# DeepRec-AI/HybridBackend

Measured on AMD Instinct MI355X. Metric: M-lookups/sec, 26-col Criteo-shape dim16, 1/2/4/8 GPUs; % HBM roofline, higher is better.
Workload: dtype f32

## Files before the change

hybridbackend_amd/csrc/common.h:

```cpp
#ifndef HBK_CSRC_COMMON_H_
#define HBK_CSRC_COMMON_H_

#include <hip/hip_runtime.h>
#include <stdarg.h>
#include <stdint.h>
#include <stdio.h>

#include "hbk.h"

namespace hbk {

int fail(int code, const char* fmt, ...);

#define HBK_HIP_OK(expr)                                                         \
  do {                                                                           \
    hipError_t e__ = (expr);                                                     \
    if (e__ != hipSuccess) {                                                     \
      return ::hbk::fail(HBK_INTERNAL, "%s failed: %s (%s:%d)", #expr,           \
                         hipGetErrorString(e__), __FILE__, __LINE__);            \
    }                                                                            \
  } while (0)

#define HBK_REQUIRE(cond, ...)                                                   \
  do {                                                                           \
// ... 45 lines not shown
  unsigned __int128 num = (unsigned __int128)1 << (64 + k);
  uint64_t m = (uint64_t)(num / d);
  uint64_t rem = (uint64_t)(num % d);
  uint64_t m2 = m * 2;
  uint64_t twice_rem = rem * 2;
  if (twice_rem >= d || twice_rem < rem) m2 += 1;
  f.magic = m2 + 1;
  f.shift = k;
  f.kind = 2;
  return f;
}

__host__ __device__ inline uint64_t mulhi64(uint64_t a, uint64_t b) {
#if defined(__HIP_DEVICE_COMPILE__)
  return __umul64hi(a, b);
#else
  return (uint64_t)(((unsigned __int128)a * b) >> 64);
#endif
}

__host__ __device__ inline uint64_t fastdiv(uint64_t n, const FastDiv& f) {
  if (f.kind == 0) return n;
  if (f.kind == 1) return n >> f.shift;
  uint64_t t = mulhi64(f.magic, n);
  return (((n - t) >> 1) + t) >> f.shift;
}

__host__ __device__ inline uint64_t fastmod(uint64_t n, const FastDiv& f) {
  if (f.kind == 0) return 0;
  if (f.kind == 1) return n & (f.d - 1);
  return n - fastdiv(n, f) * f.d;
}

__host__ __device__ inline int xcd_contiguous(int b, int n, int on) {
  if (!on) return b;
  const int q = n >> 3, r = n & 7, x = b & 7, i = b >> 3;
  return (x < r ? x * (q + 1) : r * (q + 1) + (x - r) * q) + i;
}


__host__ __device__ inline uint64_t floormod_i64(int64_t v, const FastDiv& f) {
  uint64_t u = v < 0 ? (uint64_t)(~v) : (uint64_t)v;
  uint64_t r = fastmod(u, f);
  return v < 0 ? f.d - 1 - r : r;
}

struct Options {
  int bwd_buckets_log2 = -1;
  int bwd_bucket_pairs = 0;
  int bwd_split_pairs = 0;
  int bwd_onepass = 1;
  int fwd_xcd = 1;
  int bwd_xcd = 1;
  int bwd_wide = 1;
  int bwd_group_cols = 0;
  int bwd_dense = 1;
  int bwd_scatter_staged = 1;
  int bwd_rowsort_pos = 64;
  int bwd_pairs_packed = 1;
  int bwd_seg_inline = 1;
  int bwd_scale_fused = 1;
  int bwd_deterministic = 0;
  int bwd_simple = 1;
  int bwd_streams = 4;
  int bwd_lds_pad = 0;
  int bwd_trace = 0;
  int bwd_large_first = 0;
  int bwd_rowsort_ratio = 8;
  int bwd_weights_lds = 1;
  int fwd_d16 = 1;
  int fwd_interleave = 2;
  int fwd_hot_rows = 0;
  int unique_buckets_log2 = -1;
  int partition_sub_tiles = 1;
  int partition_fixed_max = 8;
  int partition_onepass = 1;
  int unique_onepass = 1;
  int sharded_groups = 0;
  int sharded_id64 = 0;
  int sharded_copy_self = 0;
  int sharded_trace = 0;
  int sharded_pack_early = 1;
  int sharded_wire_fused = 1;
  int sharded_inline = 1;
  int sharded_p2p = 1;
  int sharded_p2p_test_refuse = -1;
  int sync_wait_ms = 2000;
  int sync_onepass_off = 0;
  int sync_test_withhold = -1;
};
Options& options();

struct SyncTake {
  int32_t* words;
  int32_t* zero;
  int64_t zero_words;
  int32_t* status;
  int32_t* summary;
  int32_t* poison;
  unsigned long long wait_ticks;
  int32_t withhold;
};
struct SyncWait {
  int32_t* status;
  int32_t* summary;
  int32_t* poison;
  unsigned long long ticks;
  int32_t withhold;
  int32_t pad_;
};
inline SyncWait sync_wait_of(const SyncTake& t) {
  SyncWait w;
  w.status = t.status;
  w.summary = t.summary;
  w.poison = t.poison;
  w.ticks = t.wait_ticks;
  w.withhold = t.withhold;
  w.pad_ = 0;
  return w;
}
#define HBK_SYNC_SAME_STREAM (reinterpret_cast<hipStream_t>(~(uintptr_t)0))
bool sync_take(hipStream_t stream, size_t words, SyncTake* out, const void* kernel = nullptr,
               int block = 0, int max_column_wgs = 0, hipStream_t owner = HBK_SYNC_SAME_STREAM);
class SyncChain {
 public:
  explicit SyncChain(hipStream_t stream);
  ~SyncChain();
  SyncChain(const SyncChain&) = delete;
  SyncChain& operator=(const SyncChain&) = delete;

 private:
  hipStream_t stream_;
  void* state_;
};
int sync_check(const char* who, hipStream_t stream);
int sync_check_any(const char* who);

struct SlotNames {
  const char* who;
  const char* opt;
  const char* s0;
  const char* s1;
};
int adam_check(const hbk_adam_t* adam, float lr, const char* who);
int ftrl_check(const hbk_ftrl_t* ftrl, float lr, const char* who);

int bwd_check(int32_t n_cols, const hbk_lookup_grad_column_t* cols, int32_t apply, float apply_lr);

struct WeightGradColumn {
  const float* table;
  int64_t rows;
  int32_t dim;
  int32_t table_pitch;
  int32_t ids_dtype;
  const void* ids;
  int64_t n_ids;
  const int32_t* row_splits;
  int64_t n_segments;
  int64_t bucket;
  int32_t divisor;
  int32_t combiner;
  const float* grad_out;
  int32_t grad_stride;
  const float* id_weights;
  float max_norm;
  float* grad_weights;
// ... 32 lines not shown
```

hybridbackend_amd/csrc/lookup_fwd.hip:

```cpp
#include <stdlib.h>
#include <string.h>

#include <vector>

#include "lookup_common.h"

namespace hbk {
namespace {

constexpr int kBlock = 256;
constexpr int kWavesPerBlock = kBlock / kWave;
constexpr int kMaxColsPerLaunch = 128;
constexpr int kU = 2;
constexpr int kSegIters = 4;

struct ColArg {
  const float* table;
  const void* ids;
  const int32_t* splits;
  float* out;
  int64_t n_seg;
  IdMap map;
  int32_t dim;
  int32_t chunks;
  uint8_t lpr_log2;
  uint8_t ids64;
  uint8_t combiner;
  uint8_t vec4;
  int32_t n_runs;
  int32_t out_stride;
  const int64_t* run_start;
  const int64_t* run_base;
  union {
    const int32_t* out_slots;
    const float* weights;
  };
};

template <bool RUNS>
__device__ inline uint64_t row_offset(const ColArg& c, uint64_t r) {
  if (!RUNS) return r * (uint64_t)c.dim;
  int k = 0;
  while (k + 1 < c.n_runs && (uint64_t)c.run_start[k + 1] <= r) ++k;
  return (uint64_t)c.run_base[k] + (r - (uint64_t)c.run_start[k]) * (uint64_t)c.dim;
}

template <typename V, int HALF>
__device__ inline void store_out_chunk(float* out, int64_t off, V v) {
  if (HALF != 1) {
    __builtin_nontemporal_store(v, reinterpret_cast<V*>(out + off));
    return;
  }
  _Float16* o = reinterpret_cast<_Float16*>(out) + off;
  if (sizeof(V) == 16) {
    const f32x4 f = *reinterpret_cast<const f32x4*>(&v);
    const f16x4 h = {(_Float16)f[0], (_Float16)f[1], (_Float16)f[2], (_Float16)f[3]};
    __builtin_nontemporal_store(h, reinterpret_cast<f16x4*>(o));
  } else {
    *o = (_Float16)*reinterpret_cast<const float*>(&v);
  }
}

struct LookupArgs {
  int32_t n_cols;
  int32_t hot_mode;
  int32_t xcd;
  int32_t interleave;
  int32_t tile_start[kMaxColsPerLaunch + 1];
  ColArg col[kMaxColsPerLaunch];
};
static_assert(sizeof(LookupArgs) <= 24576, "kernarg budget");

template <typename V, int U, bool RUNS, int HALF, bool SLOT = false, bool D16 = false, bool WGT = false,
          bool CLIP = false>
__device__ inline void gather_rows(const ColArg& c, int64_t wave_row0, float max_norm = 0.0f) {
  constexpr int VE = sizeof(V) / 4;
  const int lane = lane_id();
  const int lpr_log2 = D16 ? 2 : c.lpr_log2;
  const int rpi = kWave >> lpr_log2;
  const int sub = lane & ((1 << lpr_log2) - 1);
  const int grp = lane >> lpr_log2;
  const int64_t n_seg = c.n_seg;

  uint64_t rowreg[U];
  int32_t slotreg[U];
  float wreg[U];
  const int n_slots = U * rpi;
#pragma unroll
  for (int k = 0; k < U; ++k) {
    rowreg[k] = kNoRow;
    slotreg[k] = 0;
    wreg[k] = 0.f;
    const int q = k * kWave + lane;
    const int64_t s = wave_row0 + q;
    if (q < n_slots && s < n_seg) {
      rowreg[k] = id_to_row(c.map, load_id(c.ids, D16 ? 1 : c.ids64, s));
      if (SLOT) slotreg[k] = __builtin_nontemporal_load(c.out_slots + s);
      if (WGT) wreg[k] = __builtin_nontemporal_load(c.weights + s);
    }
  }

  V v[U];
  const bool live = D16 ? true : sub < c.chunks;
#pragma unroll
  for (int u = 0; u < U; ++u) {
    const int q0 = u * rpi;
    const int k = q0 >> 6;
    uint64_t src = rowreg[0];
#pragma unroll
    for (int kk = 1; kk < U; ++kk) src = (k == kk) ? rowreg[kk] : src;
    const uint64_t r = shfl_u64(src, (q0 & (kWave - 1)) + grp);
    v[u] = zero_v<V>();
    if (live && r != kNoRow) {
      v[u] = load_row_chunk<V, HALF>(c.table, row_offset<RUNS>(c, r) + (uint64_t)sub * VE);
    }
    if (CLIP) v[u] = clip_row<V>(v[u], max_norm, lpr_log2);
    if (WGT) {
      float w = wreg[0];
#pragma unroll
      for (int kk = 1; kk < U; ++kk) w = (k == kk) ? wreg[kk] : w;
      w = __shfl(w, (q0 & (kWave - 1)) + grp, kWave);
      const float div = c.combiner == HBK_COMBINER_MEAN    ? w
                        : c.combiner == HBK_COMBINER_SQRTN ? sqrtf(w * w)
                                                           : 1.f;
      if (r != kNoRow && div != 0.f) {
        v[u] = v[u] * w;
        if (c.combiner != HBK_COMBINER_SUM) v[u] = v[u] / div;
      } else {
        v[u] = zero_v<V>();
      }
    }
  }
#pragma unroll
  for (int u = 0; u < U; ++u) {
    const int64_t s = wave_row0 + u * rpi + grp;
    int64_t dst = s;
    if (SLOT) {
      const int q0 = u * rpi;
      const int k = q0 >> 6;
      int32_t src = slotreg[0];
#pragma unroll
      for (int kk = 1; kk < U; ++kk) src = (k == kk) ? slotreg[kk] : src;
      dst = (int64_t)__shfl(src, (q0 & (kWave - 1)) + grp, kWave);
    }
    if (live && s < n_seg) {
      store_out_chunk<V, HALF>(c.out, dst * (int64_t)c.out_stride + (int64_t)sub * VE, v[u]);
    }
  }
}

template <typename V, bool RUNS, int HALF, bool WGT = false, bool CLIP = false>
__device__ inline void combine_segments(const ColArg& c, int64_t wave_seg0, float max_norm = 0.0f) {
  constexpr int VE = sizeof(V) / 4;
  const int lane = lane_id();
  const int lpr_log2 = c.lpr_log2;
  const int lpr = 1 << lpr_log2;
  const int rpi = kWave >> lpr_log2;
  const int sub = lane & (lpr - 1);
  const int grp = lane >> lpr_log2;
  const int grp_lane0 = grp << lpr_log2;
  const int64_t n_seg = c.n_seg;
  const bool live = sub < c.chunks;

  for (int it = 0; it < kSegIters; ++it) {
    const int64_t s = wave_seg0 + (int64_t)it * rpi + grp;
    int32_t beg = 0, end = 0;
    if (s < n_seg) {
      beg = c.splits[s];
      end = c.splits[s + 1];
    }
    V acc = zero_v<V>();
    float wsum = 0.f;
    int32_t j0 = beg;
    uint64_t myrow = kNoRow;
    float myw = 0.f;
    if (j0 + sub < end) {
      myrow = id_to_row(c.map, load_id(c.ids, c.ids64, j0 + sub));
      if (WGT) myw = __builtin_nontemporal_load(c.weights + j0 + sub);
    }
    while (__any(j0 < end)) {
      uint64_t nextrow = kNoRow;
      float nextw = 0.f;
      const int32_t j1 = j0 + lpr;
      if (j1 + sub < end) {
        nextrow = id_to_row(c.map, load_id(c.ids, c.ids64, j1 + sub));
        if (WGT) nextw = __builtin_nontemporal_load(c.weights + j1 + sub);
      }
      const int32_t cnt = end - j0;
      for (int t0 = 0; t0 < lpr; t0 += 4) {
        V v[4];
        bool p[4];
        float w[4];
#pragma unroll
        for (int t = 0; t < 4; ++t) {
          const int tt = t0 + t;
          const uint64_t r = shfl_u64(myrow, grp_lane0 + (tt & (lpr - 1)));
          p[t] = tt < lpr && tt < cnt;
          if (WGT) {
            w[t] = __shfl(myw, grp_lane0 + (tt & (lpr - 1)), kWave);
            p[t] = p[t] && r != kNoRow;
          }
          v[t] = zero_v<V>();
          if (p[t] && live && r != kNoRow) {
            v[t] = load_row_chunk<V, HALF>(c.table, row_offset<RUNS>(c, r) + (uint64_t)sub * VE);
          }
          if (CLIP) v[t] = clip_row<V>(v[t], max_norm, lpr_log2);
        }
#pragma unroll
        for (int t = 0; t < 4; ++t) {
          if (WGT) {
            if (p[t]) {
              acc = acc + v[t] * w[t];
              wsum = wsum + (c.combiner == HBK_COMBINER_SQRTN ? w[t] * w[t] : w[t]);
            }
          } else {
            if (p[t]) acc = acc + v[t];
          }
        }
      }
      myrow = nextrow;
      if (WGT) myw = nextw;
      j0 = j1;
    }
    const int32_t n = end - beg;
    if (WGT) {
      if (c.combiner != HBK_COMBINER_SUM) {
        const float div = c.combiner == HBK_COMBINER_MEAN ? wsum : sqrtf(wsum);
        acc = div != 0.f ? acc / div : zero_v<V>();
      }
    } else if (n > 0 && c.combiner == HBK_COMBINER_MEAN) {
      acc = acc / (float)n;
    } else if (n > 0 && c.combiner == HBK_COMBINER_SQRTN) {
      acc = acc / sqrtf((float)n);
    }
    if (live && s < n_seg) {
      store_out_chunk<V, HALF>(c.out, s * (int64_t)c.out_stride + (int64_t)sub * VE, acc);
    }
  }
}

template <bool CSR, typename V, bool RUNS, int HALF = 0, bool SLOT = false, bool D16 = false>
__global__ __launch_bounds__(kBlock) void group_lookup_fwd_kernel(const LookupArgs a) {
  const int b = xcd_contiguous((int)blockIdx.x, (int)gridDim.x, a.xcd);
  int ci;
  int64_t tile;
  if (a.interleave) {
    ci = b % a.n_cols;
    tile = b / a.n_cols;
  } else {
    const int lane = (int)threadIdx.x & (kWave - 1);
    const int n = a.n_cols;
    const int t0 = lane < n ? a.tile_start[lane] : 0x7fffffff;
    const int t1 = lane + kWave < n ? a.tile_start[lane + kWave] : 0x7fffffff;
    ci = (int)__builtin_popcountll(__ballot(t0 <= b)) +
         (int)__builtin_popcountll(__ballot(t1 <= b)) - 1;
    ci = __builtin_amdgcn_readfirstlane(ci);
    tile = b - a.tile_start[ci];
  }
  const ColArg& c = a.col[ci];
  const int wave = (int)(threadIdx.x >> 6);
  const int rpi = D16 ? 16 : kWave >> c.lpr_log2;
  if (!CSR) {
    const int64_t row0 = (tile * kWavesPerBlock + wave) * (int64_t)(kU * rpi);
    if (row0 >= c.n_seg) return;
    gather_rows<V, kU, RUNS, HALF, SLOT, D16>(c, row0);
  } else {
    const int64_t seg0 = (tile * kWavesPerBlock + wave) * (int64_t)(kSegIters * rpi);
    if (seg0 >= c.n_seg) return;
    combine_segments<V, RUNS, HALF>(c, seg0);
  }
}

template <bool CSR, typename V, bool RUNS, int HALF>
__global__ __launch_bounds__(kBlock) void group_lookup_fwd_weighted_kernel(const LookupArgs a) {
  const int b = xcd_contiguous((int)blockIdx.x, (int)gridDim.x, a.xcd);
  int ci;
  int64_t tile;
  if (a.interleave) {
    ci = b % a.n_cols;
    tile = b / a.n_cols;
  } else {
    const int lane = (int)threadIdx.x & (kWave - 1);
    const int n = a.n_cols;
    const int t0 = lane < n ? a.tile_start[lane] : 0x7fffffff;
    const int t1 = lane + kWave < n ? a.tile_start[lane + kWave] : 0x7fffffff;
    ci = (int)__builtin_popcountll(__ballot(t0 <= b)) +
         (int)__builtin_popcountll(__ballot(t1 <= b)) - 1;
    ci = __builtin_amdgcn_readfirstlane(ci);
    tile = b - a.tile_start[ci];
  }
  const ColArg& c = a.col[ci];
  const int wave = (int)(threadIdx.x >> 6);
  const int rpi = kWave >> c.lpr_log2;
  if (!CSR) {
    const int64_t row0 = (tile * kWavesPerBlock + wave) * (int64_t)(kU * rpi);
    if (row0 >= c.n_seg) return;
    gather_rows<V, kU, RUNS, HALF, false, false, true>(c, row0);
  } else {
    const int64_t seg0 = (tile * kWavesPerBlock + wave) * (int64_t)(kSegIters * rpi);
    if (seg0 >= c.n_seg) return;
    combine_segments<V, RUNS, HALF, true>(c, seg0);
  }
}

struct ClipLookupArgs {
  LookupArgs a;
  float max_norm[kMaxColsPerLaunch];
};
static_assert(sizeof(ClipLookupArgs) <= 24576, "kernarg budget");

template <bool CSR, typename V, bool RUNS, int HALF, bool WGT>
__global__ __launch_bounds__(kBlock) void group_lookup_fwd_clip_kernel(const ClipLookupArgs ca) {
  const LookupArgs& a = ca.a;
  const int b = xcd_contiguous((int)blockIdx.x, (int)gridDim.x, a.xcd);
  int ci;
  int64_t tile;
  if (a.interleave) {
    ci = b % a.n_cols;
    tile = b / a.n_cols;
  } else {
    const int lane = (int)threadIdx.x & (kWave - 1);
    const int n = a.n_cols;
    const int t0 = lane < n ? a.tile_start[lane] : 0x7fffffff;
    const int t1 = lane + kWave < n ? a.tile_start[lane + kWave] : 0x7fffffff;
    ci = (int)__builtin_popcountll(__ballot(t0 <= b)) +
         (int)__builtin_popcountll(__ballot(t1 <= b)) - 1;
    ci = __builtin_amdgcn_readfirstlane(ci);
    tile = b - a.tile_start[ci];
  }
  const ColArg& c = a.col[ci];
  const float max_norm = ca.max_norm[ci];
  const int wave = (int)(threadIdx.x >> 6);
  const int rpi = kWave >> c.lpr_log2;
  if (!CSR) {
    const int64_t row0 = (tile * kWavesPerBlock + wave) * (int64_t)(kU * rpi);
    if (row0 >= c.n_seg) return;
    gather_rows<V, kU, RUNS, HALF, false, false, WGT, true>(c, row0, max_norm);
  } else {
    const int64_t seg0 = (tile * kWavesPerBlock + wave) * (int64_t)(kSegIters * rpi);
    if (seg0 >= c.n_seg) return;
    combine_segments<V, RUNS, HALF, WGT, true>(c, seg0, max_norm);
  }
}

constexpr int kHotTile = 256;
constexpr int kHotSlots = 1024;
constexpr int kHotStageFloats = 4096;
constexpr int kHotMaxStage = 64;
constexpr int kHotU = 4;
constexpr uint32_t kHotEmpty = 0xffffffffu;

__device__ inline uint32_t hot_mix(uint32_t k) {
  k ^= k >> 16;
// ... 110 lines not shown
          } else {
            v[u] = *reinterpret_cast<const V*>(c.table + (uint64_t)keys[q] * (uint64_t)c.dim +
                                               (uint64_t)sub * 4);
          }
        }
      }
    }
#pragma unroll
    for (int u = 0; u < kHotU; ++u) {
      const int64_t s = seg0 + s0 + u * groups + grp;
      if (s < n_seg && live) {
        __builtin_nontemporal_store(
            v[u], reinterpret_cast<V*>(c.out + s * (int64_t)c.out_stride + (int64_t)sub * 4));
      }
    }
  }
}

template <bool CSR, typename V, bool RUNS, int HALF = 0, bool SLOT = false>
void launch_kind(const LookupArgs& args, unsigned tiles, hipStream_t stream) {
  hipLaunchKernelGGL((group_lookup_fwd_kernel<CSR, V, RUNS, HALF, SLOT>), dim3(tiles), dim3(kBlock), 0,
                     stream, args);
}

template <bool CSR, typename V, bool RUNS, int HALF = 0>
void launch_weighted(const LookupArgs& args, unsigned tiles, hipStream_t stream) {
  hipLaunchKernelGGL((group_lookup_fwd_weighted_kernel<CSR, V, RUNS, HALF>), dim3(tiles), dim3(kBlock), 0,
                     stream, args);
}

constexpr int kWeightedKind = 40;
constexpr int kClipKind = 64;
constexpr int kKinds = 128;

template <bool CSR, typename V, bool RUNS, int HALF = 0, bool WGT = false>
void launch_clip(const ClipLookupArgs& args, unsigned tiles, hipStream_t stream) {
  hipLaunchKernelGGL((group_lookup_fwd_clip_kernel<CSR, V, RUNS, HALF, WGT>), dim3(tiles), dim3(kBlock), 0,
                     stream, args);
}

void launch_clip_kind(int kind, const ClipLookupArgs& args, unsigned tiles, hipStream_t stream) {
  switch (kind - kClipKind) {
    case 0: launch_clip<false, f32x4, false>(args, tiles, stream); return;
    case 1: launch_clip<true, f32x4, false>(args, tiles, stream); return;
    case 2: launch_clip<false, float, false>(args, tiles, stream); return;
    case 3: launch_clip<true, float, false>(args, tiles, stream); return;
    case 4: launch_clip<false, f32x4, true>(args, tiles, stream); return;
    case 5: launch_clip<true, f32x4, true>(args, tiles, stream); return;
    case 6: launch_clip<false, float, true>(args, tiles, stream); return;
    case 7: launch_clip<true, float, true>(args, tiles, stream); return;
    case 16: launch_clip<false, f32x4, false, 1>(args, tiles, stream); return;
    case 18: launch_clip<false, float, false, 1>(args, tiles, stream); return;
    case 32: launch_clip<false, f32x4, false, 0, true>(args, tiles, stream); return;
    case 33: launch_clip<true, f32x4, false, 0, true>(args, tiles, stream); return;
    case 34: launch_clip<false, float, false, 0, true>(args, tiles, stream); return;
    case 35: launch_clip<true, float, false, 0, true>(args, tiles, stream); return;
    case 36: launch_clip<false, f32x4, true, 0, true>(args, tiles, stream); return;
    case 37: launch_clip<true, f32x4, true, 0, true>(args, tiles, stream); return;
    case 38: launch_clip<false, float, true, 0, true>(args, tiles, stream); return;
    default: launch_clip<true, float, true, 0, true>(args, tiles, stream); return;
  }
}

void launch_by_kind(int kind, const LookupArgs& args, unsigned tiles, hipStream_t stream) {
  if (kind >= kWeightedKind) {
    switch (kind - kWeightedKind) {
      case 0: launch_weighted<false, f32x4, false>(args, tiles, stream); return;
      case 1: launch_weighted<true, f32x4, false>(args, tiles, stream); return;
      case 2: launch_weighted<false, float, false>(args, tiles, stream); return;
      case 3: launch_weighted<true, float, false>(args, tiles, stream); return;
      case 4: launch_weighted<false, f32x4, true>(args, tiles, stream); return;
      case 5: launch_weighted<true, f32x4, true>(args, tiles, stream); return;
      case 6: launch_weighted<false, float, true>(args, tiles, stream); return;
      case 7: launch_weighted<true, float, true>(args, tiles, stream); return;
      case 20: launch_weighted<false, f32x4, true, 2>(args, tiles, stream); return;
      case 21: launch_weighted<true, f32x4, true, 2>(args, tiles, stream); return;
      case 22: launch_weighted<false, float, true, 2>(args, tiles, stream); return;
      default: launch_weighted<true, float, true, 2>(args, tiles, stream); return;
    }
  }
  if (kind == 39) {
    hipLaunchKernelGGL((group_lookup_fwd_kernel<false, f32x4, false, 0, false, true>), dim3(tiles), dim3(kBlock), 0,
                       stream, args);
    return;
  }
  if (kind == 8) {
    hipLaunchKernelGGL(group_lookup_fwd_hot_kernel, dim3(tiles), dim3(kBlock), 0, stream, args);
    return;
  }
  switch (kind) {
    case 32: launch_kind<false, f32x4, false, 0, true>(args, tiles, stream); return;
    case 34: launch_kind<false, float, false, 0, true>(args, tiles, stream); return;
    case 16: launch_kind<false, f32x4, false, 1>(args, tiles, stream); return;
    case 18: launch_kind<false, float, false, 1>(args, tiles, stream); return;
    case 20: launch_kind<false, f32x4, true, 2>(args, tiles, stream); return;
    case 21: launch_kind<true, f32x4, true, 2>(args, tiles, stream); return;
    case 22: launch_kind<false, float, true, 2>(args, tiles, stream); return;
    case 23: launch_kind<true, float, true, 2>(args, tiles, stream); return;
    default: break;
  }
  switch (kind) {
    case 0: launch_kind<false, f32x4, false>(args, tiles, stream); break;
    case 1: launch_kind<true, f32x4, false>(args, tiles, stream); break;
    case 2: launch_kind<false, float, false>(args, tiles, stream); break;
    case 3: launch_kind<true, float, false>(args, tiles, stream); break;
    case 4: launch_kind<false, f32x4, true>(args, tiles, stream); break;
    case 5: launch_kind<true, f32x4, true>(args, tiles, stream); break;
    case 6: launch_kind<false, float, true>(args, tiles, stream); break;
    default: launch_kind<true, float, true>(args, tiles, stream); break;
  }
}

}
}

namespace hbk {
namespace {
int group_lookup_fwd(int32_t n_cols, const hbk_lookup_column_t* cols, const float* max_norms,
                     hbk_stream_t stream) {
  HBK_REQUIRE(n_cols >= 0, "group_lookup_fwd: n_cols must be >= 0, got %d", n_cols);
  HBK_REQUIRE(n_cols == 0 || cols != nullptr, "group_lookup_fwd: cols is NULL");
  for (int32_t c = 0; c < n_cols; ++c) {
    const hbk_lookup_column_t& h = cols[c];
    HBK_REQUIRE(h.dim >= 1, "group_lookup_fwd: column %d: dim must be >= 1, got %d", c, h.dim);
    HBK_REQUIRE(h.dim <= 1024, "group_lookup_fwd: column %d: dim %d > 1024 unsupported", c,
                h.dim);
    HBK_REQUIRE(h.rows >= 0 && h.n_ids >= 0 && h.n_segments >= 0,
                "group_lookup_fwd: column %d: negative size", c);
    HBK_REQUIRE(h.ids_dtype == HBK_INT32 || h.ids_dtype == HBK_INT64,
                "group_lookup_fwd: column %d: ids must be int32 or int64", c);
    HBK_REQUIRE(h.bucket >= 0, "group_lookup_fwd: column %d: bucket must be >= 0", c);
    HBK_REQUIRE(h.divisor >= 1, "group_lookup_fwd: column %d: divisor must be >= 1", c);
    HBK_REQUIRE(h.combiner >= HBK_COMBINER_SUM && h.combiner <= HBK_COMBINER_SQRTN,
                "group_lookup_fwd: column %d: unknown combiner %d", c, h.combiner);
    HBK_REQUIRE(h.row_splits != nullptr || h.n_segments == h.n_ids,
                "group_lookup_fwd: column %d: n_segments (%lld) must equal n_ids (%lld) "
                "when row_splits is NULL",
                c, (long long)h.n_segments, (long long)h.n_ids);
    HBK_REQUIRE(h.n_segments == 0 ||
                    ((h.table || h.rows == 0) && h.out && (h.ids || h.n_ids == 0)),
                "group_lookup_fwd: column %d: NULL buffer", c);
    HBK_REQUIRE(h.n_runs >= 0 && (h.n_runs == 0 || (h.run_start && h.run_base)),
                "group_lookup_fwd: column %d: bad segmented-table description", c);
    HBK_REQUIRE(h.n_ids < (1ll << 31) && h.n_segments < (1ll << 31),
                "group_lookup_fwd: column %d: more than 2^31-1 ids/segments", c);
    HBK_REQUIRE(h.half_io == 0 ||
                    (h.half_io == HBK_LOOKUP_OUT_HALF && h.row_splits == nullptr && h.n_runs == 0) ||
                    (h.half_io == HBK_LOOKUP_TABLE_HALF && h.n_runs > 0),
                "group_lookup_fwd: column %d: half_io %d: fp16 output rows need one id per segment "
                "and a plain table, fp16 table rows a segmented table", c, h.half_io);
    HBK_REQUIRE(h.out_slots == nullptr ||
                    (h.row_splits == nullptr && h.n_runs == 0 && h.half_io == 0),
                "group_lookup_fwd: column %d: out_slots needs one id per segment, a plain table and "
                "fp32 rows", c);
    HBK_REQUIRE(h.id_weights == nullptr || (h.out_slots == nullptr && h.half_io != HBK_LOOKUP_OUT_HALF),
                "group_lookup_fwd: column %d: id_weights cannot be combined with out_slots or "
                "HBK_LOOKUP_OUT_HALF (the owner gather is never weighted)", c);
    HBK_REQUIRE(max_norms == nullptr || max_norms[c] == 0.0f ||
                    (h.half_io != HBK_LOOKUP_TABLE_HALF && h.out_slots == nullptr),
                "group_lookup_fwd_clipped: column %d: a clipped column cannot read fp16 table rows "
                "(HBK_LOOKUP_TABLE_HALF) or write through out_slots", c);
  }

  const int hot_mode = options().fwd_hot_rows;
  struct Classified {
    RowShape shape;
    int kind;
  };
  std::vector<Classified> cls((size_t)(n_cols > 0 ? n_cols : 1));
  bool kinds_present[kKinds] = {};
  for (int32_t c = 0; c < n_cols; ++c) {
    const hbk_lookup_column_t& h = cols[c];
    cls[c].kind = -1;
    if (h.n_segments == 0) continue;
    HBK_REQUIRE(h.out_stride == 0 || h.out_stride >= h.dim,
                "group_lookup_fwd: out_stride %d is smaller than dim %d", h.out_stride, h.dim);
    const uintptr_t table_bits = (uintptr_t)h.table * (h.half_io == HBK_LOOKUP_TABLE_HALF ? 2 : 1);
    const uintptr_t out_bits = (uintptr_t)h.out * (h.half_io == HBK_LOOKUP_OUT_HALF ? 2 : 1) |
                               ((uintptr_t)(uint32_t)h.out_stride * 4);
    HBK_REQUIRE(make_rowshape(h.dim, table_bits | out_bits, &cls[c].shape),
                "group_lookup_fwd: dim %d needs more than 64 lanes per row "
                "(unaligned or dim %% 4 != 0 with dim > 64 is unsupported)", h.dim);
    const RowShape& shape = cls[c].shape;
    int col_kind = (h.row_splits != nullptr ? 1 : 0) | (shape.vec4 ? 0 : 2) |
                   (h.n_runs > 0 ? 4 : 0);
    if (h.half_io != 0) col_kind |= 16;
    if (h.out_slots != nullptr) col_kind |= 32;
    if (col_kind == 0 && (hot_mode > 0 || h.hot_rows != 0) && h.dim >= 64 && shape.lpr_log2 <= 6 &&
        h.dim <= kHotStageFloats && h.rows < 0xffffffffll) {
      col_kind = 8;
    }
    if (col_kind == 0 && options().fwd_d16 != 0 && h.dim == 16 && h.ids_dtype == HBK_INT64 && shape.lpr_log2 == 2 &&
        shape.chunks == 4) {
      col_kind = 39;
    }
    if (max_norms != nullptr && max_norms[c] != 0.0f) {
      col_kind = kClipKind + (col_kind == 8 || col_kind == 39 ? 0 : col_kind) + (h.id_weights != nullptr ? 32 : 0);
    } else if (h.id_weights != nullptr) {
      col_kind = kWeightedKind + (col_kind == 8 || col_kind == 39 ? 0 : col_kind);
    }
    cls[c].kind = col_kind;
    kinds_present[col_kind] = true;
  }
  for (int kind = 0; kind < kKinds; ++kind) {
    if (!kinds_present[kind]) continue;
    int32_t c0 = 0;
    while (c0 < n_cols) {
      LookupArgs args;
      args.hot_mode = hot_mode > 0 ? hot_mode : 1;
      args.xcd = 0;
      args.interleave = 0;
      int32_t k = 0;
      int64_t tiles = 0;
      bool same_tiles = true, one_block = true;
      uintptr_t block_lo = 0, block_hi = 0;
      int64_t small_lookups = 0, all_lookups = 0;
      float clip[kMaxColsPerLaunch];
      args.tile_start[0] = 0;
      while (c0 < n_cols && k < kMaxColsPerLaunch) {
        const int32_t ci = c0++;
        if (cls[ci].kind != kind) continue;
        const hbk_lookup_column_t& h = cols[ci];
        const RowShape& shape = cls[ci].shape;
        const int col_kind = kind;
        ColArg& d = args.col[k];
        d.table = h.table;
        d.ids = h.ids;
        d.splits = h.row_splits;
        d.out = h.out;
        d.n_seg = h.n_segments;
        d.map = make_idmap(h.bucket, h.divisor, h.rows);
        d.dim = h.dim;
        d.vec4 = shape.vec4;
        d.chunks = shape.chunks;
        d.lpr_log2 = shape.lpr_log2;
        d.ids64 = h.ids_dtype == HBK_INT64;
        d.combiner = (uint8_t)h.combiner;
        d.n_runs = h.n_runs;
        d.out_stride = h.out_stride > 0 ? h.out_stride : h.dim;
        d.run_start = h.run_start;
        d.run_base = h.run_base;
        if (kind >= kWeightedKind) {
          d.weights = h.id_weights;
        } else {
          d.out_slots = h.out_slots;
        }
        clip[k] = kind >= kClipKind ? max_norms[ci] : 0.0f;
        const int64_t rpi = kWave >> d.lpr_log2;
        const int64_t per_block =
            col_kind == 8 ? kHotTile : kWavesPerBlock * rpi * (h.row_splits ? kSegIters : kU);
        const int64_t col_tiles = (h.n_segments + per_block - 1) / per_block;
        same_tiles = same_tiles && (k == 0 || col_tiles == args.tile_start[1]);
        one_block = one_block && d.out_stride > h.dim && h.half_io == 0;
        const uintptr_t out_at = reinterpret_cast<uintptr_t>(h.out);
        block_lo = k == 0 || out_at < block_lo ? out_at : block_lo;
        block_hi = k == 0 || out_at > block_hi ? out_at : block_hi;
        one_block = one_block && (block_hi - block_lo) / sizeof(float) + (uintptr_t)h.dim <=
                                     (uintptr_t)d.out_stride;
        tiles += col_tiles;
        HBK_REQUIRE(tiles < (1ll << 31), "group_lookup_fwd: grid too large");
        all_lookups += h.n_ids;
        if (h.rows * (int64_t)h.dim * 4 <= (2ll << 20)) small_lookups += h.n_ids;
        ++k;
        args.tile_start[k] = (int32_t)tiles;
      }
      if (k == 0) continue;
      args.n_cols = k;
      const int xcd_opt = options().fwd_xcd;
      args.xcd = xcd_opt == 2 || (xcd_opt == 1 && (kind == 8 || 5 * small_lookups >= all_lookups))
                     ? 1 : 0;
      const int il = options().fwd_interleave;
      if (k > 1 && same_tiles && il > 0 &&
          (il == 3 || (one_block && (kind != 8 || il == 2)))) {
        args.interleave = 1;
      }
      if (kind >= kClipKind) {
        ClipLookupArgs ca;
// ... 34 lines not shown
```

hybridbackend_amd/csrc/misc.cpp:

```cpp
#include <stdlib.h>
#include <string.h>

#include <vector>

#include "common.h"

namespace hbk {
namespace {
thread_local char g_last_error[1024] = "";
}

int fail(int code, const char* fmt, ...) {
  va_list ap;
  va_start(ap, fmt);
  vsnprintf(g_last_error, sizeof(g_last_error), fmt, ap);
  va_end(ap);
  return code;
}
}

namespace hbk {
namespace {
struct OptionEntry {
  const char* name;
  const char* env;
  int Options::*field;
};
const OptionEntry kOptions[] = {
    {"bwd_buckets_log2", "HBK_BWD_LOG2P", &Options::bwd_buckets_log2},
    {"bwd_bucket_pairs", "HBK_BWD_TARGET", &Options::bwd_bucket_pairs},
    {"bwd_split_pairs", "HBK_BWD_SPLIT", &Options::bwd_split_pairs},
    {"bwd_onepass", "HBK_BWD_ONEPASS", &Options::bwd_onepass},
    {"bwd_group_cols", "HBK_BWD_GROUP_COLS", &Options::bwd_group_cols},
    {"bwd_dense", "HBK_BWD_DENSE", &Options::bwd_dense},
    {"bwd_scatter_staged", "HBK_BWD_SCATTER_STAGED", &Options::bwd_scatter_staged},
    {"bwd_rowsort_pos", "HBK_BWD_ROWSORT_POS", &Options::bwd_rowsort_pos},
    {"bwd_rowsort_ratio", "HBK_BWD_ROWSORT_RATIO", &Options::bwd_rowsort_ratio},
    {"bwd_deterministic", "HBK_BWD_DETERMINISTIC", &Options::bwd_deterministic},
    {"bwd_streams", "HBK_BWD_STREAMS", &Options::bwd_streams},
    {"bwd_trace", "HBK_BWD_TRACE", &Options::bwd_trace},
    {"bwd_lds_pad", "HBK_BWD_LDS_PAD", &Options::bwd_lds_pad},
    {"bwd_large_first", "HBK_BWD_LARGE_FIRST", &Options::bwd_large_first},
    {"bwd_pairs_packed", "HBK_BWD_PAIRS_PACKED", &Options::bwd_pairs_packed},
    {"bwd_seg_inline", "HBK_BWD_SEG_INLINE", &Options::bwd_seg_inline},
    {"bwd_scale_fused", "HBK_BWD_SCALE_FUSED", &Options::bwd_scale_fused},
    {"bwd_simple", "HBK_BWD_SIMPLE", &Options::bwd_simple},
    {"fwd_d16", "HBK_FWD_D16", &Options::fwd_d16},
    {"bwd_weights_lds", "HBK_BWD_WEIGHTS_LDS", &Options::bwd_weights_lds},
    {"bwd_wide", "HBK_BWD_WIDE", &Options::bwd_wide},
    {"bwd_xcd", "HBK_BWD_XCD", &Options::bwd_xcd},
    {"fwd_xcd", "HBK_FWD_XCD", &Options::fwd_xcd},
    {"fwd_hot_rows", "HBK_FWD_HOT", &Options::fwd_hot_rows},
    {"fwd_interleave", "HBK_FWD_INTERLEAVE", &Options::fwd_interleave},
    {"unique_buckets_log2", "HBK_UNIQUE_LOG2P", &Options::unique_buckets_log2},
    {"partition_sub_tiles", "HBK_PART_SUB", &Options::partition_sub_tiles},
    {"partition_fixed_max", "HBK_PART_FIXED", &Options::partition_fixed_max},
    {"partition_onepass", "HBK_PART_ONEPASS", &Options::partition_onepass},
    {"unique_onepass", "HBK_UNIQUE_ONEPASS", &Options::unique_onepass},
    {"sharded_groups", "HBK_SHARDED_GROUPS", &Options::sharded_groups},
    {"sharded_id64", "HBK_SHARDED_ID64", &Options::sharded_id64},
    {"sharded_copy_self", "HBK_SHARDED_COPY_SELF", &Options::sharded_copy_self},
    {"sharded_trace", "HBK_SHARDED_TRACE", &Options::sharded_trace},
    {"sharded_inline", "HBK_SHARDED_INLINE", &Options::sharded_inline},
    {"sharded_p2p", "HBK_SHARDED_P2P", &Options::sharded_p2p},
    {"sharded_p2p_test_refuse", "HBK_SHARDED_P2P_TEST_REFUSE", &Options::sharded_p2p_test_refuse},
    {"sharded_wire_fused", "HBK_SHARDED_WIRE_FUSED", &Options::sharded_wire_fused},
    {"sharded_pack_early", "HBK_SHARDED_PACK_EARLY", &Options::sharded_pack_early},
    {"sync_wait_ms", "HBK_SYNC_WAIT_MS", &Options::sync_wait_ms},
    {"sync_onepass_off", "HBK_SYNC_ONEPASS_OFF", &Options::sync_onepass_off},
    {"sync_test_withhold", "HBK_SYNC_TEST_WITHHOLD", &Options::sync_test_withhold},
};

Options from_environment() {
  Options o;
  for (const OptionEntry& e : kOptions) {
    const char* v = getenv(e.env);
    if (v != nullptr && *v != 0) o.*(e.field) = atoi(v);
  }
  return o;
}
}

Options& options() {
  static Options o = from_environment();
  return o;
}
}

extern "C" const char* hbk_last_error(void) { return hbk::g_last_error; }

extern "C" int hbk_set_option(const char* name, int32_t value) {
  using namespace hbk;
  HBK_REQUIRE(name != nullptr, "set_option: name is NULL");
  for (const OptionEntry& e : kOptions) {
    if (strcmp(e.name, name) == 0) {
      options().*(e.field) = value;
      return HBK_OK;
    }
  }
  return fail(HBK_INVALID_ARGUMENT, "set_option: unknown option '%s'", name);
}

extern "C" int hbk_get_option(const char* name, int32_t* value) {
  using namespace hbk;
  HBK_REQUIRE(name != nullptr && value != nullptr, "get_option: NULL argument");
  for (const OptionEntry& e : kOptions) {
    if (strcmp(e.name, name) == 0) {
      *value = options().*(e.field);
      return HBK_OK;
    }
  }
  return fail(HBK_INVALID_ARGUMENT, "get_option: unknown option '%s'", name);
}

extern "C" int hbk_sync_check(void) { return hbk::sync_check_any("sync_check"); }
extern "C" int hbk_sync_check_stream(hbk_stream_t stream) {
  return hbk::sync_check("sync_check_stream", reinterpret_cast<hipStream_t>(stream));
}

extern "C" const char* hbk_version(void) { return "hbk 0.2.0 gfx950"; }

extern "C" size_t hbk_tables_layout(int32_t n, const size_t* bytes, size_t* offsets) {
  const size_t kAlign = (size_t)2 << 20;
  size_t total = 0;
  if (n > 0 && bytes == nullptr) {
    (void)hbk::fail(HBK_INVALID_ARGUMENT, "tables_layout: bytes is NULL");
    return 0;
  }
  for (int32_t i = 0; i < n; ++i) {
    if (offsets != nullptr) offsets[i] = total;
    total += (bytes[i] + kAlign - 1) / kAlign * kAlign;
  }
  return total;
}
extern "C" int hbk_tables_alloc(int32_t n, const size_t* bytes, void** tables, void** slab) {
  using namespace hbk;
  HBK_REQUIRE(n >= 0 && (n == 0 || (bytes && tables)) && slab != nullptr,
              "tables_alloc: bad arguments");
  *slab = nullptr;
  if (n == 0) return HBK_OK;
  std::vector<size_t> off((size_t)n);
  const size_t total = hbk_tables_layout(n, bytes, off.data());
  void* p = nullptr;
  const hipError_t e = hipMalloc(&p, total > 0 ? total : 1);
  if (e != hipSuccess) {
    (void)hipGetLastError();
    return fail(HBK_INTERNAL, "tables_alloc: hipMalloc of %zu bytes failed: %s", total,
                hipGetErrorString(e));
  }
  for (int32_t i = 0; i < n; ++i) tables[i] = static_cast<char*>(p) + off[(size_t)i];
// ... 67 lines not shown
```

hybridbackend_amd/csrc/sharded.hip:

```cpp
#include <stdio.h>
#include <stdlib.h>
#include <string.h>
#include <unistd.h>

#include <algorithm>
#include <chrono>
#include <functional>
#include <random>
#include <utility>
#include <vector>

#include "common.h"

namespace hbk {
int alltoallv_events(hbk_comm_t comm, int32_t n, int32_t dtype, int32_t wire_dtype,
                     int32_t topology, const int64_t* common_sizes, const void* const* inputs,
                     const int32_t* send_sizes, void* const* outputs,
                     const int32_t* recv_sizes, void* wire_ws, size_t wire_ws_bytes,
                     hbk_stream_t compute_stream, hipEvent_t before, hipEvent_t after,
                     bool skip_self, bool inline_x);
int partition_by_modulo_fused(int32_t n_cols, int32_t num_partitions, const int64_t* const* inputs,
                              const int64_t* lens, const int64_t* buckets,
                              int64_t* const* outputs, int32_t* const* sizes,
                              int32_t* const* indices, int32_t* sizes_t, void* workspace,
// ... 83 lines not shown
    if (k == 0) continue;
    args.n_segs = k;
    hipLaunchKernelGGL(seg_copy_kernel, dim3((unsigned)tiles), dim3(kBlock), 0, stream, args);
    HBK_HIP_OK(hipGetLastError());
  }
  return HBK_OK;
}

__global__ void transpose_sizes_kernel(const int32_t* in, int32_t* out, int n, int w) {
  const int i = blockIdx.x * blockDim.x + threadIdx.x;
  if (i < n * w) out[(i % w) * n + i / w] = in[i];
}

constexpr int kSlotCols = 128;
constexpr int kSlotTile = 2048;
struct SlotArgs {
  int32_t n_cols, W, col0, pad_;
  const int64_t* shard_off;
  const int64_t* dst_off;
  int32_t* slots;
  int32_t tile0[kSlotCols + 1];
  int32_t n[kSlotCols];
  const int32_t* idx[kSlotCols];
};
static_assert(sizeof(SlotArgs) <= 16384, "kernarg budget");

__global__ __launch_bounds__(kBlock) void p2p_slots_kernel(const SlotArgs a) {
  __shared__ int64_t so[kMaxPackWorldP2p], dof[kMaxPackWorldP2p];
  int c = 0, hi = a.n_cols;
  while (hi - c > 1) {
    const int mid = (c + hi) >> 1;
    if (a.tile0[mid] <= (int)blockIdx.x) {
      c = mid;
    } else {
      hi = mid;
    }
  }
  const int W = a.W;
  for (int q = (int)threadIdx.x; q < W; q += kBlock) {
    so[q] = a.shard_off[(size_t)(a.col0 + c) * W + q];
    dof[q] = a.dst_off[(size_t)(a.col0 + c) * W + q];
  }
  __syncthreads();
  const int32_t* idx = a.idx[c];
  const int32_t n = a.n[c];
  const int32_t j0 = ((int)blockIdx.x - a.tile0[c]) * kSlotTile;
#pragma unroll
  for (int t = 0; t < kSlotTile / kBlock; ++t) {
    const int32_t j = j0 + t * kBlock + (int)threadIdx.x;
    if (j >= n) continue;
    const int64_t k = idx[j];
    int q = 0, e = W;
    while (e - q > 1) {
      const int mid = (q + e) >> 1;
      if (so[mid] <= k) {
        q = mid;
      } else {
        e = mid;
      }
    }
    a.slots[dof[q] + k - so[q]] = j;
  }
}

constexpr int kMaxPackCols = 400;
constexpr int kMaxPackWorld = 256;
constexpr int kPackTile = 2048;

struct PackArgs {
  const int32_t* S;
  void* dst;
  int64_t dst_items;
  int32_t n_cols, W, narrow, pad_;
  const int64_t* src[kMaxPackCols];
  int32_t* slots;
  const int32_t* idx[kMaxPackCols];
  int64_t gbase[kMaxPackCols];
  int32_t n[kMaxPackCols];
  int32_t tile0[kMaxPackCols];
  int16_t g0[kMaxPackCols], g1[kMaxPackCols];
};
static_assert(sizeof(PackArgs) <= 16384, "kernarg budget");

__global__ __launch_bounds__(kBlock) void pack_ids_kernel(const PackArgs a) {
  __shared__ int32_t cum[kMaxPackWorld + 1];
  __shared__ int64_t base[kMaxPackWorld];
  __shared__ int32_t peer_tot[kMaxPackWorld], before[kMaxPackWorld];
  int c = 0, hi = a.n_cols;
  while (hi - c > 1) {
    const int mid = (c + hi) >> 1;
    if (a.tile0[mid] <= (int)blockIdx.x) {
      c = mid;
    } else {
      hi = mid;
    }
  }
  const int W = a.W, tid = (int)threadIdx.x;
  if (tid < W) {
    int tot = 0, bef = 0;
    for (int cc = a.g0[c]; cc < a.g1[c]; ++cc) {
      const int s = a.S[(size_t)cc * W + tid];
      tot += s;
      if (cc < c) bef += s;
    }
    peer_tot[tid] = tot;
    before[tid] = bef;
  }
  __syncthreads();
  if (tid == 0) {
    int64_t at = a.gbase[c];
    int32_t in_col = 0;
    for (int q = 0; q < W; ++q) {
      cum[q] = in_col;
      base[q] = at + before[q];
      in_col += a.S[(size_t)c * W + q];
      at += peer_tot[q];
    }
    cum[W] = in_col;
  }
  __syncthreads();
  const int32_t n = a.n[c];
  const int64_t* src = a.src[c];
  const int32_t e0 = ((int)blockIdx.x - a.tile0[c]) * kPackTile;
#pragma unroll
  for (int k = 0; k < kPackTile / kBlock; ++k) {
    const int32_t e = e0 + k * kBlock + tid;
    if (e >= n || e >= cum[W]) break;
    const int64_t v = __builtin_nontemporal_load(src + e);
    int q = 0, qh = W;
    while (qh - q > 1) {
      const int mid = (q + qh) >> 1;
      if (cum[mid] <= e) {
        q = mid;
      } else {
        qh = mid;
      }
    }
    const int64_t at = base[q] + (e - cum[q]);
    if (at < 0 || at >= a.dst_items) continue;
    if (a.narrow) {
      reinterpret_cast<int32_t*>(a.dst)[at] = (int32_t)v;
    } else {
      reinterpret_cast<int64_t*>(a.dst)[at] = v;
    }
  }
  if (a.slots == nullptr) return;
  const int32_t* idx = a.idx[c];
#pragma unroll
  for (int k = 0; k < kPackTile / kBlock; ++k) {
    const int32_t j = e0 + k * kBlock + tid;
    if (j >= n) break;
    const int32_t e = __builtin_nontemporal_load(idx + j);
    if (e < 0 || e >= cum[W]) continue;
    int q = 0, qh = W;
    while (qh - q > 1) {
      const int mid = (q + qh) >> 1;
      if (cum[mid] <= e) {
        q = mid;
      } else {
        qh = mid;
      }
    }
    const int64_t at = base[q] + (e - cum[q]);
    if (at < 0 || at >= a.dst_items) continue;
    a.slots[at] = j;
  }
}

constexpr int kDedupTile = 2048;

struct DedupArgs {
  const int64_t* uniq;
  const int32_t* inv;
  int32_t* idx;
  const int32_t* nu;
  int32_t* S;
  int32_t* St;
  FastDiv wdiv;
  int32_t n_cols, W, N, pad_;
  int64_t off[kMaxPackCols];
  int32_t n[kMaxPackCols];
  int32_t tile0[kMaxPackCols];
  int16_t col[kMaxPackCols];
};
static_assert(sizeof(DedupArgs) <= 16384, "kernarg budget");

__global__ __launch_bounds__(kBlock) void dedup_compose_kernel(const DedupArgs a) {
  int d = 0, hi = a.n_cols;
  while (hi - d > 1) {
    const int mid = (d + hi) >> 1;
    if (a.tile0[mid] <= (int)blockIdx.x) {
      d = mid;
    } else {
      hi = mid;
    }
  }
  const int32_t n = a.n[d];
  const int32_t* inv = a.inv + a.off[d];
  int32_t* idx = a.idx + a.off[d];
  const int32_t e0 = ((int)blockIdx.x - a.tile0[d]) * kDedupTile;
#pragma unroll
  for (int k = 0; k < kDedupTile / kBlock; ++k) {
    const int32_t e = e0 + k * kBlock + (int)threadIdx.x;
    if (e < n) idx[e] = inv[idx[e]];
  }
}

__global__ __launch_bounds__(kMaxPackWorld) void dedup_sizes_kernel(const DedupArgs a) {
  __shared__ int32_t start[kMaxPackWorld + 1];
  const int d = (int)blockIdx.x, q = (int)threadIdx.x;
  const int c = a.col[d];
  const int32_t u = a.nu[c];
  const int64_t* uniq = a.uniq + a.off[d];
  if (q < a.W) {
    int32_t lo = 0, hi = u;
    while (lo < hi) {
      const int32_t mid = (lo + hi) >> 1;
      if ((int)floormod_i64(uniq[mid], a.wdiv) >= q) {
        hi = mid;
      } else {
        lo = mid + 1;
      }
    }
    start[q] = lo;
  }
  if (q == 0) start[a.W] = u;
  __syncthreads();
  if (q < a.W) {
    const int32_t cnt = start[q + 1] - start[q];
    a.S[(size_t)c * a.W + q] = cnt;
    a.St[(size_t)q * a.N + c] = cnt;
  }
}

struct Buffer {
  void* ptr = nullptr;
  size_t bytes = 0;
  int ensure(size_t need) {
    if (need <= bytes) return HBK_OK;
    if (ptr) HBK_HIP_OK(hipFree(ptr));
    ptr = nullptr;
    bytes = 0;
    const size_t grow = need + need / 4 + (1 << 20);
    HBK_HIP_OK(hipMalloc(&ptr, grow));
    bytes = grow;
// ... 1725 lines not shown
```

Before: 30000.

## Add direct stitch lookup kernel and parallelize pack_ids prefix computation

Adds a stitch_direct lookup path for sharded int32-id sum columns with few runs. Run start/offset tables are held in wave lanes and resolved with readlane, so the per-row run lookup no longer goes through memory. Separately rewrites pack_ids_kernel to issue its id and index loads before the shared-memory setup and to compute the per-shard cumulative offsets with atomics and a wave scan instead of a serial single-thread loop. The direct path adds a per-row loop over up to 16 readlanes, and the new pack code holds more registers.

New measurement: 29980, median of 4. Within noise of the previous version (-0.1%).

```diff
diff --git a/hybridbackend_amd/csrc/common.h b/hybridbackend_amd/csrc/common.h
--- a/hybridbackend_amd/csrc/common.h
+++ b/hybridbackend_amd/csrc/common.h
@@ -151,6 +151,7 @@
   int sharded_trace = 0;
   int sharded_pack_early = 1;
   int sharded_wire_fused = 1;
+  int sharded_stitch_direct = 1;
   int sharded_inline = 1;
   int sharded_p2p = 1;
   int sharded_p2p_test_refuse = -1;
diff --git a/hybridbackend_amd/csrc/lookup_fwd.hip b/hybridbackend_amd/csrc/lookup_fwd.hip
--- a/hybridbackend_amd/csrc/lookup_fwd.hip
+++ b/hybridbackend_amd/csrc/lookup_fwd.hip
@@ -45,6 +45,41 @@
   return (uint64_t)c.run_base[k] + (r - (uint64_t)c.run_start[k]) * (uint64_t)c.dim;
 }
 
+constexpr int kMaxDirectRuns = 16;
+#ifndef HBK_STITCH_NT
+#define HBK_STITCH_NT 0
+#endif
+
+struct RunRegs {
+  uint64_t start, delta;
+};
+
+__device__ inline RunRegs load_runs(const ColArg& c, int dim) {
+  RunRegs t = {0, 0};
+  const int lane = lane_id();
+  if (lane < c.n_runs) {
+    t.start = (uint64_t)c.run_start[lane];
+    t.delta = (uint64_t)c.run_base[lane] - t.start * (uint64_t)dim;
+  }
+  return t;
+}
+
+__device__ inline uint64_t readlane_u64(uint64_t v, int src_lane) {
+  const uint32_t lo = (uint32_t)__builtin_amdgcn_readlane((int)(uint32_t)v, src_lane);
+  const uint32_t hi = (uint32_t)__builtin_amdgcn_readlane((int)(uint32_t)(v >> 32), src_lane);
+  return ((uint64_t)hi << 32) | lo;
+}
+
+__device__ inline uint64_t direct_offset(const RunRegs& t, int n_runs, uint64_t r, int dim) {
+  uint64_t d = readlane_u64(t.delta, 0);
+  bool go = true;
+  for (int q = 1; q < n_runs; ++q) {
+    go = go && readlane_u64(t.start, q) <= r;
+    d = go ? readlane_u64(t.delta, q) : d;
+  }
+  return r * (uint64_t)dim + d;
+}
+
 template <typename V, int HALF>
 __device__ inline void store_out_chunk(float* out, int64_t off, V v) {
   if (HALF != 1) {
@@ -72,7 +107,7 @@
 static_assert(sizeof(LookupArgs) <= 24576, "kernarg budget");
 
 template <typename V, int U, bool RUNS, int HALF, bool SLOT = false, bool D16 = false, bool WGT = false,
-          bool CLIP = false>
+          bool CLIP = false, bool DIRECT = false>
 __device__ inline void gather_rows(const ColArg& c, int64_t wave_row0, float max_norm = 0.0f) {
   constexpr int VE = sizeof(V) / 4;
   const int lane = lane_id();
@@ -86,6 +121,9 @@
   int32_t slotreg[U];
   float wreg[U];
   const int n_slots = U * rpi;
+  const int dim = D16 ? 16 : c.dim;
+  RunRegs runs = {0, 0};
+  if (DIRECT) runs = load_runs(c, dim);
 #pragma unroll
   for (int k = 0; k < U; ++k) {
     rowreg[k] = kNoRow;
@@ -94,7 +132,7 @@
     const int q = k * kWave + lane;
     const int64_t s = wave_row0 + q;
     if (q < n_slots && s < n_seg) {
-      rowreg[k] = id_to_row(c.map, load_id(c.ids, D16 ? 1 : c.ids64, s));
+      rowreg[k] = id_to_row(c.map, load_id(c.ids, DIRECT ? 0 : D16 ? 1 : c.ids64, s));
       if (SLOT) slotreg[k] = __builtin_nontemporal_load(c.out_slots + s);
       if (WGT) wreg[k] = __builtin_nontemporal_load(c.weights + s);
     }
@@ -111,8 +149,13 @@
     for (int kk = 1; kk < U; ++kk) src = (k == kk) ? rowreg[kk] : src;
     const uint64_t r = shfl_u64(src, (q0 & (kWave - 1)) + grp);
     v[u] = zero_v<V>();
+    const uint64_t off = DIRECT ? direct_offset(runs, c.n_runs, r, dim) : 0;
     if (live && r != kNoRow) {
-      v[u] = load_row_chunk<V, HALF>(c.table, row_offset<RUNS>(c, r) + (uint64_t)sub * VE);
+      if (DIRECT && HBK_STITCH_NT) {
+        v[u] = __builtin_nontemporal_load(reinterpret_cast<const V*>(c.table + off + (uint64_t)sub * VE));
+      } else {
+        v[u] = load_row_chunk<V, HALF>(c.table, (DIRECT ? off : row_offset<RUNS>(c, r)) + (uint64_t)sub * VE);
+      }
     }
     if (CLIP) v[u] = clip_row<V>(v[u], max_norm, lpr_log2);
     if (WGT) {
@@ -269,6 +312,32 @@
     if (seg0 >= c.n_seg) return;
     combine_segments<V, RUNS, HALF>(c, seg0);
   }
+}
+
+template <bool D16>
+__global__ __launch_bounds__(kBlock) void stitch_direct_kernel(const LookupArgs a) {
+  const int b = xcd_contiguous((int)blockIdx.x, (int)gridDim.x, a.xcd);
+  int ci;
+  int64_t tile;
+  if (a.interleave) {
+    ci = b % a.n_cols;
+    tile = b / a.n_cols;
+  } else {
+    const int lane = (int)threadIdx.x & (kWave - 1);
+    const int n = a.n_cols;
+    const int t0 = lane < n ? a.tile_start[lane] : 0x7fffffff;
+    const int t1 = lane + kWave < n ? a.tile_start[lane + kWave] : 0x7fffffff;
+    ci = (int)__builtin_popcountll(__ballot(t0 <= b)) +
+         (int)__builtin_popcountll(__ballot(t1 <= b)) - 1;
+    ci = __builtin_amdgcn_readfirstlane(ci);
+    tile = b - a.tile_start[ci];
+  }
+  const ColArg& c = a.col[ci];
+  const int wave = (int)(threadIdx.x >> 6);
+  const int rpi = D16 ? 16 : kWave >> c.lpr_log2;
+  const int64_t row0 = (tile * kWavesPerBlock + wave) * (int64_t)(kU * rpi);
+  if (row0 >= c.n_seg) return;
+  gather_rows<f32x4, kU, true, 0, false, D16, false, false, true>(c, row0);
 }
 
 template <bool CSR, typename V, bool RUNS, int HALF>
@@ -545,6 +614,14 @@
   if (kind == 39) {
     hipLaunchKernelGGL((group_lookup_fwd_kernel<false, f32x4, false, 0, false, true>), dim3(tiles), dim3(kBlock), 0,
                        stream, args);
+    return;
+  }
+  if (kind == 12 || kind == 13) {
+    if (kind == 13) {
+      hipLaunchKernelGGL(stitch_direct_kernel<true>, dim3(tiles), dim3(kBlock), 0, stream, args);
+    } else {
+      hipLaunchKernelGGL(stitch_direct_kernel<false>, dim3(tiles), dim3(kBlock), 0, stream, args);
+    }
     return;
   }
   if (kind == 8) {
@@ -656,6 +733,11 @@
     if (col_kind == 0 && options().fwd_d16 != 0 && h.dim == 16 && h.ids_dtype == HBK_INT64 && shape.lpr_log2 == 2 &&
         shape.chunks == 4) {
       col_kind = 39;
+    }
+    const bool clipped = max_norms != nullptr && max_norms[c] != 0.0f;
+    if (col_kind == 4 && options().sharded_stitch_direct != 0 && h.n_runs <= kMaxDirectRuns &&
+        h.ids_dtype == HBK_INT32 && h.combiner == HBK_COMBINER_SUM && h.id_weights == nullptr && !clipped) {
+      col_kind = h.dim == 16 && shape.lpr_log2 == 2 && shape.chunks == 4 ? 13 : 12;
     }
     if (max_norms != nullptr && max_norms[c] != 0.0f) {
       col_kind = kClipKind + (col_kind == 8 || col_kind == 39 ? 0 : col_kind) + (h.id_weights != nullptr ? 32 : 0);
diff --git a/hybridbackend_amd/csrc/misc.cpp b/hybridbackend_amd/csrc/misc.cpp
--- a/hybridbackend_amd/csrc/misc.cpp
+++ b/hybridbackend_amd/csrc/misc.cpp
@@ -66,6 +66,7 @@
     {"sharded_p2p_test_refuse", "HBK_SHARDED_P2P_TEST_REFUSE", &Options::sharded_p2p_test_refuse},
     {"sharded_wire_fused", "HBK_SHARDED_WIRE_FUSED", &Options::sharded_wire_fused},
     {"sharded_pack_early", "HBK_SHARDED_PACK_EARLY", &Options::sharded_pack_early},
+    {"sharded_stitch_direct", "HBK_SHARDED_STITCH_DIRECT", &Options::sharded_stitch_direct},
     {"sync_wait_ms", "HBK_SYNC_WAIT_MS", &Options::sync_wait_ms},
     {"sync_onepass_off", "HBK_SYNC_ONEPASS_OFF", &Options::sync_onepass_off},
     {"sync_test_withhold", "HBK_SYNC_TEST_WITHHOLD", &Options::sync_test_withhold},
diff --git a/hybridbackend_amd/csrc/sharded.hip b/hybridbackend_amd/csrc/sharded.hip
--- a/hybridbackend_amd/csrc/sharded.hip
+++ b/hybridbackend_amd/csrc/sharded.hip
@@ -189,85 +189,120 @@
 };
 static_assert(sizeof(PackArgs) <= 16384, "kernarg budget");
 
+__device__ inline int pack_shard_of(const int32_t* cum, int W, int32_t e) {
+  int q = 0, qh = W;
+  while (qh - q > 1) {
+    const int mid = (q + qh) >> 1;
+    if (cum[mid] <= e) {
+      q = mid;
+    } else {
+      qh = mid;
+    }
+  }
+  return q;
+}
+
 __global__ __launch_bounds__(kBlock) void pack_ids_kernel(const PackArgs a) {
+  constexpr int kPer = kPackTile / kBlock;
   __shared__ int32_t cum[kMaxPackWorld + 1];
   __shared__ int64_t base[kMaxPackWorld];
   __shared__ int32_t peer_tot[kMaxPackWorld], before[kMaxPackWorld];
-  int c = 0, hi = a.n_cols;
-  while (hi - c > 1) {
-    const int mid = (c + hi) >> 1;
-    if (a.tile0[mid] <= (int)blockIdx.x) {
-      c = mid;
-    } else {
-      hi = mid;
-    }
-  }
-  const int W = a.W, tid = (int)threadIdx.x;
-  if (tid < W) {
-    int tot = 0, bef = 0;
-    for (int cc = a.g0[c]; cc < a.g1[c]; ++cc) {
-      const int s = a.S[(size_t)cc * W + tid];
-      tot += s;
-      if (cc < c) bef += s;
-    }
-    peer_tot[tid] = tot;
-    before[tid] = bef;
-  }
-  __syncthreads();
-  if (tid == 0) {
-    int64_t at = a.gbase[c];
-    int32_t in_col = 0;
-    for (int q = 0; q < W; ++q) {
-      cum[q] = in_col;
-      base[q] = at + before[q];
-      in_col += a.S[(size_t)c * W + q];
-      at += peer_tot[q];
-    }
-    cum[W] = in_col;
-  }
-  __syncthreads();
+  __shared__ int32_t wave_own[kBlock / kWave];
+  __shared__ int64_t wave_tot[kBlock / kWave];
+  const int W = a.W, tid = (int)threadIdx.x, lane = tid & (kWave - 1), wave = tid >> 6;
+  int c = -1;
+  for (int i0 = 0; i0 < a.n_cols; i0 += kWave) {
+    const int t0 = i0 + lane < a.n_cols ? a.tile0[i0 + lane] : 0x7fffffff;
+    c += (int)__builtin_popcountll(__ballot(t0 <= (int)blockIdx.x));
+  }
+  c = __builtin_amdgcn_readfirstlane(c);
   const int32_t n = a.n[c];
   const int64_t* src = a.src[c];
+  const int32_t* idx = a.idx[c];
   const int32_t e0 = ((int)blockIdx.x - a.tile0[c]) * kPackTile;
+  const bool slots = a.slots != nullptr;
+  const int g0 = a.g0[c], g1 = a.g1[c];
+  const int32_t own = tid < W ? a.S[(size_t)c * W + tid] : 0;
+  const int group_items = (g1 - g0) * W;
+  const int32_t* Sg = a.S + (size_t)g0 * W;
+  const int32_t s_first = tid < group_items ? Sg[tid] : 0;
+  int64_t v[kPer];
+  int32_t ix[kPer];
 #pragma unroll
-  for (int k = 0; k < kPackTile / kBlock; ++k) {
+  for (int k = 0; k < kPer; ++k) {
     const int32_t e = e0 + k * kBlock + tid;
-    if (e >= n || e >= cum[W]) break;
-    const int64_t v = __builtin_nontemporal_load(src + e);
-    int q = 0, qh = W;
-    while (qh - q > 1) {
-      const int mid = (q + qh) >> 1;
-      if (cum[mid] <= e) {
-        q = mid;
-      } else {
-        qh = mid;
-      }
-    }
+    v[k] = e < n ? __builtin_nontemporal_load(src + e) : 0;
+  }
+  if (slots) {
+#pragma unroll
+    for (int k = 0; k < kPer; ++k) {
+      const int32_t j = e0 + k * kBlock + tid;
+      ix[k] = j < n ? __builtin_nontemporal_load(idx + j) : -1;
+    }
+  }
+  if (tid < W) {
+    peer_tot[tid] = 0;
+    before[tid] = 0;
+  }
+  __syncthreads();
+  for (int i = tid; i < group_items; i += kBlock) {
+    const int32_t s = i == tid ? s_first : Sg[i];
+    const int cc = i / W, q = i - cc * W;
+    atomicAdd(&peer_tot[q], s);
+    if (g0 + cc < c) atomicAdd(&before[q], s);
+  }
+  __syncthreads();
+  const int64_t tot = tid < W ? (int64_t)peer_tot[tid] : 0;
+  int32_t own_incl = own;
+  int64_t tot_incl = tot;
+#pragma unroll
+  for (int o = 1; o < kWave; o <<= 1) {
+    const int32_t x = __shfl_up(own_incl, o, kWave);
+    const int64_t y = (int64_t)__shfl_up((long long)tot_incl, o, kWave);
+    if (lane >= o) {
+      own_incl += x;
+      tot_incl += y;
+    }
+  }
+  if (lane == kWave - 1) {
+    wave_own[wave] = own_incl;
+    wave_tot[wave] = tot_incl;
+  }
+  __syncthreads();
+  int32_t own_excl = own_incl - own;
+  int64_t tot_excl = tot_incl - tot;
+  for (int w = 0; w < wave; ++w) {
+    own_excl += wave_own[w];
+    tot_excl += wave_tot[w];
+  }
+  if (tid < W) {
+    cum[tid] = own_excl;
+    base[tid] = a.gbase[c] + tot_excl + before[tid];
+  }
+  if (tid == W - 1) cum[W] = own_excl + own;
+  __syncthreads();
+  const int32_t n_live = cum[W] < n ? cum[W] : n;
+#pragma unroll
+  for (int k = 0; k < kPer; ++k) {
+    const int32_t e = e0 + k * kBlock + tid;
+    if (e >= n_live) break;
+    const int q = pack_shard_of(cum, W, e);
     const int64_t at = base[q] + (e - cum[q]);
     if (at < 0 || at >= a.dst_items) continue;
     if (a.narrow) {
-      reinterpret_cast<int32_t*>(a.dst)[at] = (int32_t)v;
+      reinterpret_cast<int32_t*>(a.dst)[at] = (int32_t)v[k];
     } else {
-      reinterpret_cast<int64_t*>(a.dst)[at] = v;
-    }
-  }
-  if (a.slots == nullptr) return;
-  const int32_t* idx = a.idx[c];
+      reinterpret_cast<int64_t*>(a.dst)[at] = v[k];
+    }
+  }
+  if (!slots) return;
 #pragma unroll
-  for (int k = 0; k < kPackTile / kBlock; ++k) {
+  for (int k = 0; k < kPer; ++k) {
     const int32_t j = e0 + k * kBlock + tid;
     if (j >= n) break;
-    const int32_t e = __builtin_nontemporal_load(idx + j);
+    const int32_t e = ix[k];
     if (e < 0 || e >= cum[W]) continue;
-    int q = 0, qh = W;
-    while (qh - q > 1) {
-      const int mid = (q + qh) >> 1;
-      if (cum[mid] <= e) {
-        q = mid;
-      } else {
-        qh = mid;
-      }
-    }
+    const int q = pack_shard_of(cum, W, e);
     const int64_t at = base[q] + (e - cum[q]);
     if (at < 0 || at >= a.dst_items) continue;
     a.slots[at] = j;
```
